# HIPS/DESI-MCMC

Hardware: AMD Instinct MI355X
Metric: source-pixel evals/sec + full-field log-lik ms, 10k sources x 5 bands x 2048^2 (higher is better)
Workload: dtype f64

## Files before the change

### desi-mcmc_amd/csrc/celeste_hip.hip

```cpp

#include <hip/hip_runtime.h>
#include <hip/hip_ext.h>

#include <cmath>
#include <cstdarg>
#include <cstddef>
#include <cstdint>
#include <cstdio>
#include <cstring>
#include <algorithm>
#include <atomic>
#include <memory>
#include <new>
#include <vector>
#include <type_traits>

#include "../../include/celeste_hip.h"
#include "host_buf.h"

static thread_local char g_err[512] = "";

static int fail(int code, const char *fmt, ...) {
    va_list ap;
    va_start(ap, fmt);
    vsnprintf(g_err, sizeof(g_err), fmt, ap);
    va_end(ap);
    return code;
}

#define HIP_TRY(expr)                                                                         \
    do {                                                                                      \
        hipError_t e_ = (expr);                                                               \
        if (e_ != hipSuccess) {                                                               \
            (void)hipDeviceSynchronize();                                                     \
            return fail(e_ == hipErrorOutOfMemory ? CEL_ERR_NOMEM : CEL_ERR_HIP, "%s: %s (%s:%d)", \
                        #expr, hipGetErrorString(e_), __FILE__, __LINE__);                    \
        }                                                                                     \
    } while (0)

#include "device_common.h"
#include "k_prep_bin.h"
#include "k_bin2.h"
#include "k_render.h"
#include "k_render_hw.h"
#include "k_render_stars.h"
#include "k_small_stars.h"
#include "k_border.h"
#include "k_render_qw.h"
#include "k_misc.h"
#include "k_patch_ll.h"
#include "k_slice_gen.h"
#include "k_estep.h"
#include "k_grad.h"
#include "k_split.h"
#include "k_slice.h"

struct Prof {
    static const int PAIRS = 1024;
    hipEvent_t *ev = nullptr;
    int kid[PAIRS];
    int head = 0, count = 0;
    double sum_ms[CEL_K_COUNT] = {0};
    int64_t n[CEL_K_COUNT] = {0};
    unsigned seen[CEL_K_COUNT] = {0};
};

enum ScratchSlot {
    SCR_PLL_BOXES,
    SCR_OFFSETS,
    SCR_VALUES,
    SCR_PATCH_DATA,
    SCR_TMP_A,
    SCR_TMP_B,
    SCR_TMP_C,
    SCR_HOST_IO,
    SCR_COUNT
};
static_assert(SCR_COUNT == 8, "eight scratch slots");

union MailShared {
    unsigned long long bin_coarse[2];
    int64_t scan_total;
    int slice_flags[12];
    struct {
        unsigned long long flags_[3];
        unsigned long long slice_bytes;
        double field_stats[2];
    } w;
};
struct Mailbox {
    double ll_band[MAX_BANDS];
    unsigned long long bin_fine[2];
    MailShared sh;
    int slice_flags1[12];
    int mass_todo;
    int unused_[3];
};
static_assert(sizeof(Mailbox) == sizeof(double) * (MAX_BANDS + 16), "the mailbox is MAX_BANDS + 16 doubles");
static_assert(offsetof(Mailbox, bin_fine) == sizeof(double) * MAX_BANDS && offsetof(Mailbox, sh) == sizeof(double) * (MAX_BANDS + 2) &&
              offsetof(MailShared, w.slice_bytes) == sizeof(int) * 6 && offsetof(MailShared, w.field_stats) == sizeof(double) * 4 &&
              offsetof(Mailbox, slice_flags1) == sizeof(double) * (MAX_BANDS + 8) && offsetof(Mailbox, mass_todo) == sizeof(double) * (MAX_BANDS + 14),
              "the mailbox members keep their offsets");
static_assert(offsetof(Mailbox, mass_todo) >= offsetof(Mailbox, slice_flags1) + sizeof(int) * 11 && sizeof(MailShared) <= sizeof(double) * 6,
              "the pending to-do count shares no word: flag slot 1 ends before it, the shared words before flag slot 1");

#ifndef SLICE_FUSE_DEFAULT
#define SLICE_FUSE_DEFAULT 0
#endif
struct cel_ctx {
    int device = 0;
    hipStream_t stream = nullptr;
    bool own_stream = false;
    int variant = 1;
    static bool env_tail_ok() { const char *e = getenv("CEL_TAIL_LOG"); return e && atof(e) >= 0.0 && atof(e) <= 300.0; }
    double tail_T = env_tail_ok() ? atof(getenv("CEL_TAIL_LOG")) : 32.0;
    double render_T = env_tail_ok() ? atof(getenv("CEL_TAIL_LOG")) : 24.0;
    int live = 0;
    int split_full = 0;
    int slice_fuse = SLICE_FUSE_DEFAULT;
    int incremental = (getenv("CEL_INCREMENTAL") && atoi(getenv("CEL_INCREMENTAL")) == 0) ? 0 : 1;
    int tile_parts = (getenv("CEL_TILE_PARTS") && (atoi(getenv("CEL_TILE_PARTS")) == 1 || atoi(getenv("CEL_TILE_PARTS")) == 2 || atoi(getenv("CEL_TILE_PARTS")) == 4))
                         ? atoi(getenv("CEL_TILE_PARTS")) : 0;
    int profile = 0;
    int star_tiles = (getenv("CEL_STAR_TILES") && atoi(getenv("CEL_STAR_TILES")) >= 0 && atoi(getenv("CEL_STAR_TILES")) <= 3)
                         ? atoi(getenv("CEL_STAR_TILES")) : 1;
    int n_cu = 256;
    int tile_order = 1;
    int tile_rows = 32;
    bool tile_timing = false;
    double nz_bias = getenv("CEL_NZ_BIAS") ? atof(getenv("CEL_NZ_BIAS")) : 4.0;
    int split_reuse = getenv("CEL_SPLIT_REUSE") ? std::min(std::max(atoi(getenv("CEL_SPLIT_REUSE")), 0), 2) : 2;
    bool mass_reuse_of() const { return split_reuse >= 2; }
    int nz_force = 0;
    int debug = 0;
    int tile_layout = 1;
    Prof prof;
    PinnedBuf<Mailbox> mail;
    hipEvent_t slice_ev[2] = {nullptr, nullptr};
    DevBuf<char> scratch[SCR_COUNT];
};

static int scratch_get(cel_ctx *c, ScratchSlot slot, size_t bytes, void **out) {
    if (bytes == 0) bytes = 8;
    HIP_TRY(c->scratch[slot].grow(bytes, bytes + bytes / 2 + 256, c->stream));
    *out = c->scratch[slot];
    return CEL_OK;
}

struct SourcesDeleter {
    void operator()(cel_sources *s) const { cel_sources_destroy(s); }
};

struct cel_images {
    cel_ctx *ctx = nullptr;
    int B = 0, H = 0, W = 0;
    int full_H = 0, win_y0 = 0;
    int noise_y0 = 0, noise_y1 = 0x7fffffff;
    int TW = 64, TH = 32, ntx = 0, nty = 0;
    cel_band hb[MAX_BANDS];
    DevBuf<BandDev> d_bands;
    DevBuf<double> d_nelec, d_lambda, d_partials, d_llband;
    bool have_nelec = false;
    DevBuf<double> d_slabs;
    DevBuf<int> d_part_cnt;
    DevBuf<SrcRec> d_recs;
    DevBuf<int4> d_boxes;
    DevBuf<int> d_kind;
    DevBuf<int> d_status;
    uint64_t recs_gen = 0, hbox_gen = 0;
    uint64_t lambda_gen = 0, lists_gen = 0;
    DevBuf<unsigned long long> d_massfx;
    uint64_t massfx_gen = 0;
    DevBuf<int> d_mass_todo;
    std::vector<int4> h_boxes;
    std::vector<int> h_status;
    DevBuf<int> d_tile_cnt, d_tile_nstar, d_tile_work, d_order;
    DevBuf<int> d_tile_cost;
    int64_t cost_S = -1;
    bool bin_two_level = false;
    int64_t mass_pending = -1;
    int64_t mass_todo_S = -1;
    uint64_t mass_gen = 0;
    const int *mass_todo_ptr = nullptr;
    double *d_mass = nullptr;
    DevBuf<long long> d_btot;
    bool nelec_u16 = false;
    bool star_one_segment = false;
    int64_t order_S = -1;
    hipEvent_t ev_step = nullptr;
    DevBuf<int64_t> d_tile_off;
    unsigned long long *d_cursor = nullptr;
    DevBuf<int> d_lists;
    int nsx = 0, nsy = 0;
    DevBuf<int> d_sup_cnt;
    DevBuf<int64_t> d_sup_off;
    DevBuf<int> d_clist;
    DevBuf<unsigned long long> d_timing;
    DevBuf<int> d_samp;
    bool ssum_valid = false;
    PinnedBuf<double> h_ssum;
    PinnedBuf<int64_t> h_soff;
    bool hsum_valid = false;
    DevBuf<NzEntry> d_nzlist;
    bool nz_valid = false;
    DevBuf<double> d_rate;
    bool rate_in_lambda = false;
    DevBuf<int4> d_sbox;
    DevBuf<int4> d_snz;
    DevBuf<int64_t> d_soff;
    DevBuf<double> d_ssum;
    DevBuf<int> d_nnz, d_nzmode;
    DevBuf<int64_t> d_nzoff;
    int64_t samp_S = 0, samp_total = 0;
    DevBuf<double> d_stats;
    DevBuf<char> d_slice;
    std::unique_ptr<cel_sources, SourcesDeleter> slice_prop;
    DevBuf<char> d_sgen;
    std::unique_ptr<cel_sources, SourcesDeleter> sgen_prop;
    int64_t last_S = 0;
    double last_entries = 0;
    bool counted = false;
    bool nelec_shared = false;
    uint64_t partials_gen = 0;
    uint64_t lambda_uid = 0;
    double lambda_T = -1.0;
    int lambda_parts = 0;
    DevBuf<int> d_dirty;
    int64_t last_dirty = -1;
    MappedBuf<double> h_small;
    double *d_small = nullptr;
    DevBuf<double> d_small_consts;
    unsigned long long small_seq = 0;
    bool llband_on_host = false;
    double h_llband[MAX_BANDS] = {0};
    bool small_off = false;
};

static std::atomic<uint64_t> g_source_gen{0};

struct cel_sources {
    cel_ctx *ctx = nullptr;
    bool counted = false;
    int64_t cap = 0, S = 0;
    int B = 0;
    uint64_t gen = 0;
    uint64_t uid = 0;
    uint64_t full_gen = 0;
    std::vector<uint64_t> row_gen;
    int64_t n_gal = -1;
    DevBuf<int> d_type;
    DevBuf<double> d_radec, d_counts, d_shape;
    std::vector<int32_t> h_type;
};

static inline int tile_parts_of(const cel_ctx *c, const cel_images *im) {
    if (im->TW != 32 || c->variant == 0) return 1;
    if (c->tile_parts) return c->tile_parts;
    const int64_t T = (int64_t)im->B * im->ntx * im->nty;
    return T <= 512 ? 4 : (T <= 3072 ? 2 : 1);
}
static inline int tile_order_of(const cel_ctx *c, const cel_images *im) {
    return ((int64_t)im->B * im->ntx * im->nty * tile_parts_of(c, im) > 2048) ? c->tile_order : 0;
}

static bool prof_alloc(Prof &p) {
    if (p.ev) return true;
    p.ev = (hipEvent_t *)calloc(2 * Prof::PAIRS, sizeof(hipEvent_t));
    if (!p.ev) return false;
    for (int i = 0; i < 2 * Prof::PAIRS; i++)
        if (hipEventCreate(&p.ev[i]) != hipSuccess) return false;
    return true;
}
static bool prof_harvest_one(Prof &p, bool wait) {
    if (p.count == 0) return false;
    const int t = (p.head - p.count + Prof::PAIRS) % Prof::PAIRS;
    if (wait) (void)hipEventSynchronize(p.ev[2 * t + 1]);
    else if (hipEventQuery(p.ev[2 * t + 1]) != hipSuccess) return false;
    float ms = 0.f;
    if (hipEventElapsedTime(&ms, p.ev[2 * t], p.ev[2 * t + 1]) == hipSuccess) {
        p.sum_ms[p.kid[t]] += ms;
        p.n[p.kid[t]] += 1;
    }
    p.count--;
    return true;
}
static int prof_slot(cel_ctx *c, int k) {
    if (!c->profile) return -1;
    if (c->profile >= 2 && (k == CEL_K_PREP || k == CEL_K_BIN || k == CEL_K_REDUCE)) return -1;
    if (c->profile == 3 && (c->prof.seen[k]++ & 3) != 0) return -1;
    Prof &p = c->prof;
    if (!prof_alloc(p)) return -1;
    if (p.count == Prof::PAIRS) prof_harvest_one(p, true);
    else if (p.count > Prof::PAIRS / 2) { if (prof_harvest_one(p, false)) prof_harvest_one(p, false); }
    const int t = p.head;
    p.head = (p.head + 1) % Prof::PAIRS;
    p.count++;
    p.kid[t] = k;
    return 2 * t;
}
static int prof_begin(cel_ctx *c, int k) {
    const int i = prof_slot(c, k);
    if (i >= 0) (void)hipEventRecord(c->prof.ev[i], c->stream);
    return i;
}
static void prof_end(cel_ctx *c, int i) {
    if (i >= 0) (void)hipEventRecord(c->prof.ev[i + 1], c->stream);
}
#define EV0(c, i) ((i) >= 0 ? (c)->prof.ev[(i)] : (hipEvent_t) nullptr)
#define EV1(c, i) ((i) >= 0 ? (c)->prof.ev[(i) + 1] : (hipEvent_t) nullptr)
template <class T> static inline T ext_arg(const T &v) { return v; }
template <class T, unsigned F> static inline T *ext_arg(const Buf<T, F> &b) { return b.get(); }
template <class K, class... A>
static inline void ext_launch(K kernel, dim3 grid, dim3 block, hipStream_t st, hipEvent_t e0, hipEvent_t e1, const A &...a) {
// ... 159 lines not shown
    case CEL_OPT_KERNEL:
        if (v != 0.0 && v != 1.0) return fail(CEL_ERR_INVALID, "CEL_OPT_KERNEL must be 0 or 1");
        c->variant = (int)v;
        return CEL_OK;
    case CEL_OPT_TAIL_LOG:
        if (v != v) { c->tail_T = 32.0; c->render_T = 24.0; return CEL_OK; }
        if (!(v >= 0.0) || v > 300.0) return fail(CEL_ERR_INVALID, "CEL_OPT_TAIL_LOG must be in [0, 300] (NaN: the defaults)");
        c->tail_T = v;
        c->render_T = v;
        return CEL_OK;
    case CEL_OPT_TAIL_LOG_SOURCE:
        if (v != v) { c->tail_T = 32.0; return CEL_OK; }
        if (!(v >= 0.0) || v > 300.0) return fail(CEL_ERR_INVALID, "CEL_OPT_TAIL_LOG_SOURCE must be in [0, 300] (NaN: the default)");
        c->tail_T = v;
        return CEL_OK;
    case CEL_OPT_INCREMENTAL:
        if (v != 0.0 && v != 1.0) return fail(CEL_ERR_INVALID, "CEL_OPT_INCREMENTAL must be 0 or 1");
        c->incremental = (int)v;
        return CEL_OK;
    case CEL_OPT_SPLIT_FULL_BOX:
        if (v != 0.0 && v != 1.0) return fail(CEL_ERR_INVALID, "CEL_OPT_SPLIT_FULL_BOX must be 0 or 1");
        c->split_full = (int)v;
        return CEL_OK;
    case CEL_OPT_SLICE_FUSE:
        if (!(v >= 0.0 && v <= 1e9) || v != floor(v)) return fail(CEL_ERR_INVALID, "CEL_OPT_SLICE_FUSE must be 0, 1 or a block count");
        c->slice_fuse = (int)v;
        return CEL_OK;
    case CEL_OPT_TILE_PARTS:
        if (v != 0.0 && v != 1.0 && v != 2.0 && v != 4.0) return fail(CEL_ERR_INVALID, "CEL_OPT_TILE_PARTS must be 0 (by the frame's size), 1, 2 or 4");
        c->tile_parts = (int)v;
        return CEL_OK;
    case CEL_OPT_PROFILE:
        if (v != 0.0 && v != 1.0 && v != 2.0 && v != 3.0) return fail(CEL_ERR_INVALID, "CEL_OPT_PROFILE must be 0, 1, 2 or 3");
        if (v != 0.0 && !prof_alloc(c->prof)) return fail(CEL_ERR_HIP, "CEL_OPT_PROFILE: cannot create the timing events");
        c->profile = (int)v;
        return CEL_OK;
    case CEL_OPT_TILE_ORDER:
        if (v != 0.0 && v != 1.0 && v != 2.0) return fail(CEL_ERR_INVALID, "CEL_OPT_TILE_ORDER must be 0, 1 or 2");
        c->tile_order = (int)v;
        return CEL_OK;
    case CEL_OPT_TILE_ROWS:
        if (v != 32.0 && v != 64.0) return fail(CEL_ERR_INVALID, "CEL_OPT_TILE_ROWS must be 32 or 64");
        c->tile_rows = (int)v;
        return CEL_OK;
    case CEL_OPT_TILE_TIMING:
        c->tile_timing = (v != 0.0);
        return CEL_OK;
    case CEL_OPT_TILE_LAYOUT:
        if (v != 0.0 && v != 1.0 && v != 2.0) return fail(CEL_ERR_INVALID, "CEL_OPT_TILE_LAYOUT must be 0, 1 or 2");
        c->tile_layout = (int)v;
        return CEL_OK;
    case CEL_OPT_PHOTON_LISTS:
        if (v != 0.0 && v != 1.0 && v != 2.0) return fail(CEL_ERR_INVALID, "CEL_OPT_PHOTON_LISTS must be 0, 1 or 2");
        c->nz_force = (int)v;
        return CEL_OK;
    case CEL_OPT_SPLIT_REUSE:
        if (v != 0.0 && v != 1.0 && v != 2.0) return fail(CEL_ERR_INVALID, "CEL_OPT_SPLIT_REUSE must be 0, 1 or 2");
        c->split_reuse = (int)v;
        return CEL_OK;
    case CEL_OPT_STAR_TILES:
        if (v != 0.0 && v != 1.0 && v != 2.0 && v != 3.0) return fail(CEL_ERR_INVALID, "CEL_OPT_STAR_TILES must be 0, 1, 2 or 3");
        c->star_tiles = (int)v;
        return CEL_OK;
    case CEL_OPT_DEBUG:
        if (!(v >= 0.0) || v > 4095.0) return fail(CEL_ERR_INVALID, "CEL_OPT_DEBUG must be in [0, 4095]");
#ifndef CEL_ABLATE
        if (((int)v) & ~(64 | 128))
            return fail(CEL_ERR_INVALID, "CEL_OPT_DEBUG: the timing-only ablation bits exist only in a -DCEL_ABLATE build "
                                         "(make -C desi-mcmc_amd/csrc ablate); this library accepts 64 and 128");
#endif
        c->debug = (int)v;
        return CEL_OK;
    }
    return fail(CEL_ERR_INVALID, "unknown option %d", key);
}

int cel_ctx_get_option(cel_ctx *c, int key, double *v) {
    if (!c || !v) return fail(CEL_ERR_INVALID, "null argument");
    switch (key) {
    case CEL_OPT_KERNEL: *v = c->variant; return CEL_OK;
    case CEL_OPT_TAIL_LOG: *v = c->render_T; return CEL_OK;
    case CEL_OPT_TAIL_LOG_SOURCE: *v = c->tail_T; return CEL_OK;
    case CEL_OPT_TILE_PARTS: *v = c->tile_parts; return CEL_OK;
    case CEL_OPT_INCREMENTAL: *v = c->incremental; return CEL_OK;
    case CEL_OPT_SPLIT_FULL_BOX: *v = c->split_full; return CEL_OK;
    case CEL_OPT_SLICE_FUSE: *v = c->slice_fuse; return CEL_OK;
    case CEL_OPT_PROFILE: *v = (double)c->profile; return CEL_OK;
    case CEL_OPT_TILE_ORDER: *v = (double)c->tile_order; return CEL_OK;
    case CEL_OPT_TILE_ROWS: *v = c->tile_rows; return CEL_OK;
    case CEL_OPT_TILE_TIMING: *v = c->tile_timing ? 1.0 : 0.0; return CEL_OK;
    case CEL_OPT_TILE_LAYOUT: *v = c->tile_layout; return CEL_OK;
    case CEL_OPT_PHOTON_LISTS: *v = c->nz_force; return CEL_OK;
    case CEL_OPT_STAR_TILES: *v = c->star_tiles; return CEL_OK;
    case CEL_OPT_SPLIT_REUSE: *v = c->split_reuse; return CEL_OK;
    case CEL_OPT_DEBUG: *v = c->debug; return CEL_OK;
    }
    return fail(CEL_ERR_INVALID, "unknown option %d", key);
}

int cel_images_destroy(cel_images *im) {
    if (!im) return CEL_OK;
    (void)hipSetDevice(im->ctx->device);
    (void)hipStreamSynchronize(im->ctx->stream);
    if (im->ev_step) (void)hipEventDestroy(im->ev_step);
    if (im->counted) im->ctx->live--;
    delete im;
    return CEL_OK;
}

int cel_images_create(cel_ctx *c, int B, int H, int W, const cel_band *bands, cel_images **out) {
    if (!c || !bands || !out) return fail(CEL_ERR_INVALID, "cel_images_create: null argument");
    if (B < 1 || B > MAX_BANDS) return fail(CEL_ERR_INVALID, "B=%d out of range [1,%d]", B, MAX_BANDS);
    if (H < 1 || W < 1 || (int64_t)H * W > (int64_t)1 << 34) return fail(CEL_ERR_INVALID, "bad image size %dx%d", H, W);
    HIP_TRY(hipSetDevice(c->device));
    std::unique_ptr<cel_images> im(new (std::nothrow) cel_images());
    if (!im) return fail(CEL_ERR_NOMEM, "out of host memory");
    im->ctx = c; im->B = B; im->H = H; im->W = W;
    im->full_H = H; im->win_y0 = 0;
    if (c->tile_layout == 1) { im->TW = HW_TW; im->TH = HW_TH; }
    else if (c->tile_layout == 2) { im->TW = QW_TW; im->TH = QW_TH; }
    else { im->TW = TILE_W; im->TH = c->tile_rows; }
    im->ntx = (W + im->TW - 1) / im->TW;
    im->nty = (H + im->TH - 1) / im->TH;
    im->nsx = (W + SUPER_W - 1) / SUPER_W;
    im->nsy = (H + SUPER_H - 1) / SUPER_H;
    BandDev hb[MAX_BANDS];
    for (int b = 0; b < B; b++) {
        im->hb[b] = bands[b];
        for (int k = 0; k < K_PSF; k++) {
            const double *cv = bands[b].cov + 4 * k;
            double det = cv[0] * cv[3] - cv[1] * cv[2];
            if (!(cv[0] > 0) || !(cv[3] > 0) || !(det > 0))
                return fail(CEL_ERR_INVALID, "band %d: PSF component %d covariance is not positive definite", b, k);
        }
        if (!(im->hb[b].R > 0.0))
            im->hb[b].R = host_bounding_radius(bands[b].mu, bands[b].cov, K_PSF, 0.001, nullptr);
        band_to_dev(im->hb[b], hb[b]);
    }
    im->star_one_segment = true;
    for (int b = 0; b < B; b++)
        for (int k = 0; k < K_PSF; k++) {
            const BandDev &d = hb[b];
            const double inv = 1.0 / (d.cxx[k] * d.cyy[k] - d.cxy[k] * d.cxy[k]);
            const double rb_ = d.R + 2.0;
            const double emax = 0.5 * quad_max_rect_hw(d.cyy[k] * inv, -d.cxy[k] * inv, d.cxx[k] * inv, -rb_ - d.mux[k], rb_ - d.mux[k],
                                                       -rb_ - d.muy[k], rb_ - d.muy[k]);
            if (!(emax <= 0.999 * STAR_EMAX)) im->star_one_segment = false;
        }
    const int64_t npix = (int64_t)B * H * W;
    const int T = B * im->ntx * im->nty, NS = B * im->nsx * im->nsy;
    hipStream_t st = c->stream;
    HIP_TRY(im->d_bands.grow(B, B, st));
    HIP_TRY(hipMemcpy(im->d_bands, hb, sizeof(BandDev) * B, hipMemcpyHostToDevice));
    HIP_TRY(im->d_nelec.grow(npix, npix, st));
    HIP_TRY(im->d_lambda.grow(npix, npix, st));
    HIP_TRY(im->d_partials.grow(T, T, st));
    HIP_TRY(im->d_llband.grow(MAX_BANDS + 4, MAX_BANDS + 4, st));
    im->d_cursor = reinterpret_cast<unsigned long long *>(im->d_llband + MAX_BANDS);
    HIP_TRY(im->d_tile_cnt.grow(T, T, st));
    HIP_TRY(im->d_tile_nstar.grow(T, T, st));
    HIP_TRY(im->d_tile_work.grow(T, T, st));
    HIP_TRY(im->d_tile_cost.grow(T, T, st));
    HIP_TRY(im->d_order.grow(T, T, st));
    HIP_TRY(im->d_tile_off.grow(T, T, st));
    HIP_TRY(im->d_sup_cnt.grow(NS, NS, st));
    HIP_TRY(im->d_sup_off.grow(NS, NS, st));
    HIP_TRY(im->d_stats.grow(2, 2, st));
    HIP_TRY(hipMemsetAsync(im->d_lambda, 0, sizeof(double) * npix, st));
    im->counted = true;
    c->live++;
    *out = im.release();
    return CEL_OK;
}

int cel_images_set_nelec(cel_images *im, const double *nelec, int mem) {
    if (!im || !nelec) return fail(CEL_ERR_INVALID, "cel_images_set_nelec: null argument");
    HIP_TRY(hipSetDevice(im->ctx->device));
    int rc = copy_in(im->d_nelec, nelec, sizeof(double) * (size_t)im->B * im->H * im->W, mem, im->ctx->stream);
    if (rc != CEL_OK) return rc;
    im->have_nelec = true;
    im->partials_gen = 0;
    im->nelec_u16 = false;
    {
        const int NB = 512;
        DevBuf<double> d_rng;
        HIP_TRY(d_rng.grow(3 * NB, 3 * NB, im->ctx->stream));
        hipLaunchKernelGGL(k_nelec_range, dim3(NB), dim3(256), 0, im->ctx->stream, (const double *)im->d_nelec,
                           (int64_t)im->B * im->H * im->W, d_rng);
        std::vector<double> h((size_t)3 * NB);
        HIP_TRY(hipMemcpyAsync(h.data(), d_rng, sizeof(double) * 3 * NB, hipMemcpyDeviceToHost, im->ctx->stream));
        HIP_TRY(hipStreamSynchronize(im->ctx->stream));
        double lo = INFINITY, hi = -INFINITY, bad = 0.0;
        for (int k = 0; k < NB; k++) { lo = fmin(lo, h[3 * k]); hi = fmax(hi, h[3 * k + 1]); bad += h[3 * k + 2]; }
        im->nelec_u16 = (bad == 0.0) && (lo >= 0.0) && (hi <= 65535.0);
    }
    return CEL_OK;
}

int cel_images_set_epsilon(cel_images *im, int band, double eps) {
    if (!im || band < 0 || band >= im->B) return fail(CEL_ERR_INVALID, "cel_images_set_epsilon: bad band");
    HIP_TRY(hipSetDevice(im->ctx->device));
    im->hb[band].eps = eps;
    im->lambda_gen = 0;
    im->partials_gen = 0;
    hipLaunchKernelGGL(k_set_eps, dim3(1), dim3(1), 0, im->ctx->stream, im->d_bands, band, eps);
    HIP_TRY(hipGetLastError());
    return CEL_OK;
}

int cel_images_set_window(cel_images *im, int y0, int full_H) {
    if (!im) return fail(CEL_ERR_INVALID, "null images");
    if (y0 < 0 || full_H < 1 || (int64_t)y0 + im->H > full_H)
        return fail(CEL_ERR_INVALID, "window rows [%d, %d) do not fit a %d-row frame", y0, y0 + im->H, full_H);
    im->win_y0 = y0;
    im->full_H = full_H;
    im->recs_gen = im->hbox_gen = 0;
    im->lambda_gen = im->lists_gen = 0;
    im->massfx_gen = 0;
    return CEL_OK;
}

int cel_images_set_noise_rows(cel_images *im, int y0, int y1) {
    if (!im) return fail(CEL_ERR_INVALID, "null images");
    if (y0 < 0 || y1 < y0) return fail(CEL_ERR_INVALID, "cel_images_set_noise_rows: rows [%d, %d)", y0, y1);
    im->noise_y0 = y0;
    im->noise_y1 = y1;
    return CEL_OK;
}

int cel_images_get_band(cel_images *im, int band, cel_band *out) {
    if (!im || !out || band < 0 || band >= im->B) return fail(CEL_ERR_INVALID, "cel_images_get_band: bad argument");
    *out = im->hb[band];
    return CEL_OK;
}

int cel_images_get_lambda(cel_images *im, double *out, int mem) {
    if (!im || !out) return fail(CEL_ERR_INVALID, "cel_images_get_lambda: null argument");
    HIP_TRY(hipSetDevice(im->ctx->device));
    return copy_out(out, im->d_lambda, sizeof(double) * (size_t)im->B * im->H * im->W, mem, im->ctx->stream);
}

int cel_images_device_ptrs(cel_images *im, void **nelec, void **lambda) {
    if (!im) return fail(CEL_ERR_INVALID, "null images");
    if (nelec) {
        *nelec = im->d_nelec; im->nelec_u16 = false; im->nelec_shared = true; im->partials_gen = 0;
    }
    if (lambda) *lambda = im->d_lambda;
    return CEL_OK;
}

int cel_images_loglik_device(cel_images *im, void **ll_band) {
    if (!im || !ll_band) return fail(CEL_ERR_INVALID, "cel_images_loglik_device: null argument");
    if (im->llband_on_host) {
        cel_ctx *c = im->ctx;
        HIP_TRY(hipSetDevice(c->device));
        HIP_TRY(hipMemcpyAsync(im->d_llband, im->h_llband, sizeof(double) * im->B, hipMemcpyHostToDevice, c->stream));
        HIP_TRY(hipStreamSynchronize(c->stream));
        im->llband_on_host = false;
    }
    *ll_band = im->d_llband;
    return CEL_OK;
}

int cel_sources_destroy(cel_sources *s) {
    if (!s) return CEL_OK;
    (void)hipSetDevice(s->ctx->device);
    (void)hipStreamSynchronize(s->ctx->stream);
    if (s->counted) s->ctx->live--;
    delete s;
    return CEL_OK;
}

int cel_sources_create(cel_ctx *c, int64_t capacity, int B, cel_sources **out) {
    if (!c || !out) return fail(CEL_ERR_INVALID, "cel_sources_create: null argument");
    if (capacity < 1 || capacity > ((int64_t)1 << 30)) return fail(CEL_ERR_INVALID, "bad capacity");
    if (B < 1 || B > MAX_BANDS) return fail(CEL_ERR_INVALID, "B=%d out of range", B);
    HIP_TRY(hipSetDevice(c->device));
    std::unique_ptr<cel_sources> s(new (std::nothrow) cel_sources());
    if (!s) return fail(CEL_ERR_NOMEM, "out of host memory");
    s->ctx = c; s->cap = capacity; s->B = B;
    s->uid = ++g_source_gen;
    HIP_TRY(s->d_type.grow(capacity, capacity, c->stream));
    HIP_TRY(s->d_radec.grow(2 * capacity, 2 * capacity, c->stream));
    HIP_TRY(s->d_counts.grow(B * capacity, B * capacity, c->stream));
    HIP_TRY(s->d_shape.grow(4 * capacity, 4 * capacity, c->stream));
    s->counted = true;
    s->ctx->live++;
    *out = s.release();
    return CEL_OK;
}

int cel_sources_set(cel_sources *s, int64_t S, const int32_t *type, const double *radec,
                    const double *counts, const double *shape, int mem) {
    if (!s || !type || !radec || !counts || !shape) return fail(CEL_ERR_INVALID, "cel_sources_set: null argument");
    if (S < 0 || S > s->cap) return fail(CEL_ERR_INVALID, "S=%lld exceeds capacity %lld", (long long)S, (long long)s->cap);
    HIP_TRY(hipSetDevice(s->ctx->device));
    hipStream_t st = s->ctx->stream;
    if (S > 0) {
        const hipMemcpyKind kind = (mem == CEL_DEVICE) ? hipMemcpyDeviceToDevice : hipMemcpyHostToDevice;
        HIP_TRY(hipMemcpyAsync(s->d_type, type, sizeof(int) * S, kind, st));
        HIP_TRY(hipMemcpyAsync(s->d_radec, radec, sizeof(double) * 2 * S, kind, st));
        HIP_TRY(hipMemcpyAsync(s->d_counts, counts, sizeof(double) * s->B * S, kind, st));
        HIP_TRY(hipMemcpyAsync(s->d_shape, shape, sizeof(double) * 4 * S, kind, st));
        if (mem != CEL_DEVICE) HIP_TRY(hipStreamSynchronize(st));
    }
    s->S = S;
    s->gen = s->full_gen = ++g_source_gen;
    s->row_gen.clear();
    s->n_gal = -1;
    s->h_type.clear();
    if (mem != CEL_DEVICE) {
        s->n_gal = 0;
        for (int64_t i = 0; i < S; i++) s->n_gal += (type[i] != 0);
        s->h_type.assign(type, type + S);
    }
    return CEL_OK;
}

int cel_sources_get(cel_sources *s, int32_t *type, double *radec, double *counts, double *shape) {
    if (!s) return fail(CEL_ERR_INVALID, "cel_sources_get: null argument");
    HIP_TRY(hipSetDevice(s->ctx->device));
    hipStream_t st = s->ctx->stream;
    const int64_t S = s->S;
    if (S > 0) {
        if (type) HIP_TRY(hipMemcpyAsync(type, s->d_type, sizeof(int) * S, hipMemcpyDeviceToHost, st));
        if (radec) HIP_TRY(hipMemcpyAsync(radec, s->d_radec, sizeof(double) * 2 * S, hipMemcpyDeviceToHost, st));
        if (counts) HIP_TRY(hipMemcpyAsync(counts, s->d_counts, sizeof(double) * s->B * S, hipMemcpyDeviceToHost, st));
        if (shape) HIP_TRY(hipMemcpyAsync(shape, s->d_shape, sizeof(double) * 4 * S, hipMemcpyDeviceToHost, st));
        HIP_TRY(hipStreamSynchronize(st));
    }
    return CEL_OK;
}

int cel_sources_set_rows(cel_sources *s, int64_t n, const int32_t *idx, const int32_t *type, const double *radec,
                         const double *counts, const double *shape) {
    if (!s || n < 0 || (n > 0 && (!idx || !type || !radec || !counts || !shape)))
        return fail(CEL_ERR_INVALID, "cel_sources_set_rows: null argument");
    for (int64_t i = 0; i < n; i++)
        if (idx[i] < 0 || idx[i] >= s->S) return fail(CEL_ERR_INVALID, "cel_sources_set_rows: row %d outside the catalogue's %lld", idx[i], (long long)s->S);
    if (n == 0) return CEL_OK;
    {
        std::vector<int32_t> seen(idx, idx + n);
        std::sort(seen.begin(), seen.end());
        for (int64_t i = 1; i < n; i++)
            if (seen[i] == seen[i - 1]) return fail(CEL_ERR_INVALID, "cel_sources_set_rows: row %d is named twice", seen[i]);
    }
    cel_ctx *c = s->ctx;
    HIP_TRY(hipSetDevice(c->device));
    hipStream_t st = c->stream;
    const int B = s->B;
    const size_t ints = ((size_t)(2 * n) * sizeof(int) + 7) & ~(size_t)7;
    const size_t bytes = ints + sizeof(double) * (size_t)n * (2 + B + 4);
    char *d = nullptr;
    int rc = scratch_get(c, SCR_HOST_IO, bytes, (void **)&d);
    if (rc) return rc;
    std::vector<char> h(bytes);
    memcpy(h.data(), idx, sizeof(int) * n);
    memcpy(h.data() + sizeof(int) * n, type, sizeof(int) * n);
    double *hd = reinterpret_cast<double *>(h.data() + ints);
    memcpy(hd, radec, sizeof(double) * 2 * n);
    memcpy(hd + 2 * n, counts, sizeof(double) * B * n);
    memcpy(hd + (2 + B) * n, shape, sizeof(double) * 4 * n);
    HIP_TRY(hipMemcpyAsync(d, h.data(), bytes, hipMemcpyHostToDevice, st));
    const double *dd = reinterpret_cast<const double *>(d + ints);
    hipLaunchKernelGGL(k_scatter_rows, dim3((unsigned)((n + 255) / 256)), dim3(256), 0, st, n, B, (const int *)d, (const int *)d + n,
                       dd, dd + 2 * n, dd + (2 + B) * n, s->d_type, s->d_radec, s->d_counts, s->d_shape);
    HIP_TRY(hipGetLastError());
    HIP_TRY(hipStreamSynchronize(st));
    if ((int64_t)s->h_type.size() == s->S) {
        for (int64_t i = 0; i < n; i++) {
            s->n_gal += (type[i] != 0) - (s->h_type[idx[i]] != 0);
            s->h_type[idx[i]] = type[i];
        }
    } else {
        s->n_gal = -1;
    }
    s->gen = ++g_source_gen;
    if ((int64_t)s->row_gen.size() != s->S) s->row_gen.assign((size_t)s->S, 0);
    for (int64_t i = 0; i < n; i++) s->row_gen[idx[i]] = s->gen;
    return CEL_OK;
}

static int ensure_recs(cel_images *im, int64_t n) {
    if (n <= im->d_recs.cap) return CEL_OK;
    im->recs_gen = im->hbox_gen = 0;
    const int64_t cap = n + n / 4 + 64;
    HIP_TRY(grow_group(im->ctx->stream, im->d_boxes, cap, im->d_kind, cap, im->d_status, cap, im->d_recs, cap));
    return CEL_OK;
}

static double rsq_galaxy() {
    double q = 1.0 - 1e-5;
    return -2.0 * log1p(-q);
}

static int run_prep(cel_images *im, cel_sources *src, const int *d_live = nullptr, int nobox = 0) {
    cel_ctx *c = im->ctx;
    int64_t n = src->S * im->B;
    int rc = ensure_recs(im, n > 0 ? n : 1);
    if (rc) return rc;
    if (n == 0) { im->recs_gen = src->gen; im->last_S = 0; return CEL_OK; }
    int pi = prof_slot(c, CEL_K_PREP);
    LAUNCH_EV(k_prep, dim3((unsigned)((n + 255) / 256)), dim3(256), c->stream, EV0(c, pi), EV1(c, pi), im->d_bands, im->B,
              im->full_H, im->W, im->win_y0, im->H, src->S, src->d_type, src->d_radec, src->d_counts, src->d_shape,
              rsq_galaxy(), im->d_recs, im->d_boxes, im->d_kind, im->d_status, im->d_cursor, d_live, nobox);
    HIP_TRY(hipGetLastError());
    im->recs_gen = (d_live || nobox) ? 0 : src->gen;
    im->last_S = src->S;
    return CEL_OK;
}

static int host_boxes(cel_images *im, cel_sources *src) {
    if (im->hbox_gen == src->gen && src->gen != 0 && im->recs_gen == src->gen) return CEL_OK;
    int rc = CEL_OK;
    if (im->recs_gen != src->gen || src->gen == 0) rc = run_prep(im, src);
    if (rc) return rc;
    const int64_t n = src->S * im->B;
    im->h_boxes.resize((size_t)n);
    im->h_status.resize((size_t)n);
    if (n) {
        hipStream_t st = im->ctx->stream;
        HIP_TRY(hipMemcpyAsync(im->h_boxes.data(), im->d_boxes, sizeof(int4) * n, hipMemcpyDeviceToHost, st));
        HIP_TRY(hipMemcpyAsync(im->h_status.data(), im->d_status, sizeof(int) * n, hipMemcpyDeviceToHost, st));
        HIP_TRY(hipStreamSynchronize(st));
    }
    im->hbox_gen = src->gen;
    return CEL_OK;
}

#define CEL_RENDER_STRICT 4
#define CEL_RENDER_KEEP_LISTS 16
static int render_impl(cel_images *im, cel_sources *src, int flags, double *ll_band, double *ll_total, double *lambda_out);

int cel_render_field(cel_images *im, cel_sources *src, int flags, double *ll_band, double *ll_total) {
    if (flags & ~(CEL_RENDER_LOGLIK | CEL_RENDER_NO_STORE)) return fail(CEL_ERR_INVALID, "cel_render_field: unknown flag bits");
    return render_impl(im, src, flags, ll_band, ll_total, nullptr);
}

static int render_small_stars(cel_images *im, cel_sources *src, int flags, bool *done) {
    cel_ctx *c = im->ctx;
    hipStream_t st = c->stream;
    const int64_t S = src->S;
    const int B = im->B;
    *done = false;
    int rc = ensure_recs(im, S * B);
    if (rc) return rc;
    const int nblk = B * im->ntx * im->nty * SMALL_NB, nblk_band = im->ntx * im->nty * SMALL_NB;
    if (!im->h_small) {
        HIP_TRY(im->h_small.grow(nblk + 1, nblk + 1, st));
        memset(im->h_small, 0, sizeof(double) * (nblk + 1));
        HIP_TRY(hipHostGetDevicePointer((void **)&im->d_small, im->h_small, 0));
        HIP_TRY(im->d_small_consts.grow(SMALL_CONSTS * B, SMALL_CONSTS * B, st));
        hipLaunchKernelGGL(k_small_consts, dim3(B), dim3(64), 0, st, (const BandDev *)im->d_bands, im->d_small_consts);
    }
    RenderArgs a;
    memset(&a, 0, sizeof(a));
    a.bands = im->d_bands; a.recs = im->d_recs; a.nelec = im->d_nelec; a.lambda = im->d_lambda; a.partials = im->d_small;
    a.S = S; a.B = B; a.H = im->H; a.W = im->W; a.ntx = im->ntx; a.nty = im->nty;
    a.flags = flags; a.variant = c->variant; a.tail_T = c->render_T;
    SmallArgs x;
    x.radec = src->d_radec; x.counts = src->d_counts;
    x.recs = im->d_recs; x.boxes = im->d_boxes; x.kind = im->d_kind; x.status = im->d_status;
    x.partials = im->d_small;
    x.flag = reinterpret_cast<unsigned long long *>(im->d_small + nblk);
    x.stamp = 0x8000000000000000ull | ++im->small_seq;
    x.full_H = im->full_H; x.win_y0 = im->win_y0;
    x.consts = im->d_small_consts;
    {
        int mul = (int)(nblk_band * 0.381966) | 1;
        auto gcd = [](int a, int b) { while (b) { int t = a % b; a = b; b = t; } return a; };
        while (mul > 1 && gcd(mul, nblk_band) != 1) mul += 2;
        if (nblk_band < 4) mul = 1;
        x.perm_mul = mul % nblk_band ? mul % nblk_band : 1;
        x.perm_add = nblk_band / 3 + 1;
    }
    x.stamps = nullptr;
    static const char *stamp_path = getenv("CEL_SMALL_STAMPS");
    DevBuf<unsigned long long> d_stamps;
    if (stamp_path) { HIP_TRY(d_stamps.grow(8 * nblk, 8 * nblk, st)); x.stamps = d_stamps; }
    int pi = prof_slot(c, CEL_K_SMALL_STARS);
    LAUNCH_EV(k_small_stars, dim3((unsigned)nblk), dim3(64 * SMALL_NWV), st, EV0(c, pi), EV1(c, pi), a, x);
    const bool ll = (flags & CEL_RENDER_LOGLIK) != 0;
    HIP_TRY(hipGetLastError());
    HIP_TRY(hipStreamSynchronize(st));
    if (d_stamps) {
        std::vector<unsigned long long> hs((size_t)8 * nblk);
        (void)hipMemcpy(hs.data(), d_stamps, sizeof(unsigned long long) * 8 * nblk, hipMemcpyDeviceToHost);
        if (FILE *fp = fopen(stamp_path, "wb")) { fwrite(hs.data(), sizeof(unsigned long long), hs.size(), fp); fclose(fp); }
    }
    unsigned long long cur0;
    memcpy(&cur0, im->h_small + nblk, sizeof(cur0));
    if (cur0 == x.stamp) { im->small_off = true; return CEL_OK; }
    if (ll) {
        for (int b = 0; b < B; b++) {
            const double *pb = im->h_small + (size_t)b * nblk_band;
            double sum[8] = {0, 0, 0, 0, 0, 0, 0, 0}, comp[8] = {0, 0, 0, 0, 0, 0, 0, 0};
            int i = 0;
            for (; i + 8 <= nblk_band; i += 8)
                for (int k = 0; k < 8; k++) {
                    const double y = pb[i + k] - comp[k];
                    const double t = sum[k] + y;
                    comp[k] = (t - sum[k]) - y;
                    sum[k] = t;
                }
            for (int k = 0; i < nblk_band; i++, k++) {
                const double y = pb[i] - comp[k];
                const double t = sum[k] + y;
                comp[k] = (t - sum[k]) - y;
                sum[k] = t;
            }
            c->mail->ll_band[b] = ((sum[0] + sum[1]) + (sum[2] + sum[3])) + ((sum[4] + sum[5]) + (sum[6] + sum[7]));
            im->h_llband[b] = c->mail->ll_band[b];
        }
        im->llband_on_host = true;
    }
    im->recs_gen = src->gen;
    im->lists_gen = 0;
    if (!(flags & CEL_RENDER_NO_STORE)) im->lambda_gen = 0;
    im->last_S = S;
    im->cost_S = -1; im->order_S = -1;
    im->last_entries = 0;
    *done = true;
    return CEL_OK;
}

struct RenderPlan {
    int flags;
    bool keep_lists, own_rows;
    int own_ty0, own_ty1;
    bool diag, stars_only;
    bool small_stars, incremental;
    int parts, parts_used;
    int tile_order;
    bool bin_direct;
};

static int plan_render(const cel_images *im, const cel_sources *src, int flags, const double *lambda_out, RenderPlan &p) {
    const cel_ctx *c = im->ctx;
    const int64_t S = src->S;
    const int T = im->B * im->ntx * im->nty;
    p.keep_lists = (flags & CEL_RENDER_KEEP_LISTS) != 0;
    p.flags = flags &= ~CEL_RENDER_KEEP_LISTS;
    p.own_rows = im->noise_y0 > 0 || im->noise_y1 < im->H;
    p.own_ty0 = 0; p.own_ty1 = im->nty;
    if (p.own_rows && (flags & CEL_RENDER_LOGLIK)) {
        if (im->noise_y0 % im->TH != 0 || (im->noise_y1 % im->TH != 0 && im->noise_y1 < im->H))
            return fail(CEL_ERR_INVALID, "the owned rows [%d, %d) must begin and end on render-tile rows (%d) for a log-likelihood",
                        im->noise_y0, im->noise_y1, im->TH);
        p.own_ty0 = im->noise_y0 / im->TH;
        p.own_ty1 = std::min(im->nty, (im->noise_y1 + im->TH - 1) / im->TH);
    }
    p.diag = c->tile_timing || (c->debug & ~64);
    const bool stars = im->TW == HW_TW && !p.diag && c->variant != 0 && src->n_gal == 0 && im->star_one_segment;
    p.stars_only = stars && c->star_tiles && (c->star_tiles == 2 || T > STAR_TILES_MIN);
    p.small_stars = stars && S > 0 && S <= SMALL_MAX_S && T <= STAR_TILES_MIN && c->star_tiles == 1 && !im->small_off && !lambda_out &&
                    !p.keep_lists && !(flags & CEL_RENDER_STRICT) && !p.own_rows;
// ... 1544 lines not shown
```

### desi-mcmc_amd/csrc/k_prep_bin.h

```cpp
#pragma once
#include "device_common.h"
__device__ inline void dev_pixel2equa(const BandDev &b, double x, double y, double cphi, double &ra,
                                      double &dec) {
    double d0 = x - b.rho[0], d1 = y - b.rho[1];
    double i0 = b.ups[0] * d0 + b.ups[1] * d1;
    double i1 = b.ups[2] * d0 + b.ups[3] * d1;
    ra = i0 / cphi + b.phi[0];
    dec = i1 + b.phi[1];
}

__device__ inline double clampd(double v, double lo, double hi) { return fmin(fmax(v, lo), hi); }

__device__ inline double comp_radius(double cxx, double cxy, double cyy, double rsq_inv, double dist) {
    double s1 = sqrt(cxx), s2 = sqrt(cyy);
    double rho = cxy / (s1 * s2);
    double A11 = s1, A21 = rho * s2, A22 = s2 * sqrt(1.0 - rho * rho);
    double An = rsq_inv * (1.0 / (A11 * A11) + (A21 * A21) / (A22 * A22));
    double Bn = rsq_inv * (-2.0 * A21 / (A11 * (A22 * A22)));
    double Cn = rsq_inv * 1.0 / (A22 * A22);
    double maj = 1.0 / sqrt(0.5 * (An + Cn - sqrt(Bn * Bn + (An - Cn) * (An - Cn))));
    return maj + dist;
}

__device__ __forceinline__ void prep_pixel(const BandDev &bd, double ra, double dec, double cphi, double &px, double &py) {
    double s0 = (ra - bd.phi[0]) * cphi, s1 = dec - bd.phi[1];
    px = (bd.ups_inv[0] * s0 + bd.ups_inv[1] * s1) + bd.rho[0];
    py = (bd.ups_inv[2] * s0 + bd.ups_inv[3] * s1) + bd.rho[1];
}

__device__ __forceinline__ void prep_star_box(const BandDev &bd, double px, double py, int H, int W, SrcRec &r) {
    const double BIG = 1073741824.0;
    bool miss = (px < -50 || px > 2.0 * H || py < -50 || px > 2.0 * W);
    if (miss || !(px == px) || !(py == py)) {
        r.type = -3;
    } else {
        double bound = bd.R;
        int lx = (int)clampd(px - bound, -BIG, BIG), hx = (int)clampd(px + bound + 1, -BIG, BIG);
        int ly = (int)clampd(py - bound, -BIG, BIG), hy = (int)clampd(py + bound + 1, -BIG, BIG);
        r.x0 = max(0, lx); r.x1 = min(hx, W);
        r.y0 = max(0, ly); r.y1 = min(hy, H);
    }
}

__device__ __forceinline__ void prep_window(SrcRec &r, double py, int win_y0, int win_h) {
    r.y0 = max(r.y0, win_y0) - win_y0;
    r.y1 = min(r.y1, win_y0 + win_h) - win_y0;
    r.py = py - (double)win_y0;
    if (r.type < 0 || r.x1 <= r.x0 || r.y1 <= r.y0) {
        r.x0 = r.x1 = r.y0 = r.y1 = 0;
        if (r.type >= 0) r.type = -1 - r.type;
    }
}

__device__ __forceinline__ void prep_store(const SrcRec &r, int64_t i, SrcRec *__restrict__ recs, int4 *__restrict__ boxes,
                                           int *__restrict__ kind, int *__restrict__ status) {
    recs[i] = r;
    boxes[i] = make_int4(r.x0, r.x1, r.y0, r.y1);
    kind[i] = r.type < 0 ? 0 : (r.type == 0 ? K_PSF : K_GAL);
    status[i] = r.type >= 0 ? 1 : (r.type == -3 ? -1 : 0);
}

struct PrepArgs {
    const BandDev *bands;
    int B, H, W, win_y0, win_h;
    int64_t S;
    const int *type;
    const double *counts, *shape;
    double rsq_gal;
    SrcRec *recs; int4 *boxes; int *kind; int *status;
    int nobox;
};
__device__ __forceinline__ void prep_one(const BandDev *__restrict__ bands, int b, int64_t s, int64_t i, int B, int H, int W, int win_y0, int win_h,
                                         const int *__restrict__ type, double ra, double dec, const double *__restrict__ counts,
                                         const double *__restrict__ shape, double rsq_gal, SrcRec *__restrict__ recs,
                                         int4 *__restrict__ boxes, int *__restrict__ kind, int *__restrict__ status, int nobox) {
    const BandDev &bd = bands[b];
    SrcRec r;
    memset(&r, 0, sizeof(r));
    int t = type[s];
    double cphi = cos(bd.phi[1] / 180.0 * PI_D);
    double px, py;
    prep_pixel(bd, ra, dec, cphi, px, py);
    r.px = px; r.py = py;
    r.scale = counts[s * B + b];
    r.type = t;
    const double BIG = 1073741824.0;
    if (t == 0) {
        prep_star_box(bd, px, py, H, W, r);
    } else if (t == 1) {
        double theta = shape[4 * s], sig = shape[4 * s + 1], phi_s = shape[4 * s + 2], rho_s = shape[4 * s + 3];
        double ra0, dec0, rax, decx, ray, decy;
        dev_pixel2equa(bd, px, py, cphi, ra0, dec0);
        dev_pixel2equa(bd, px + 10.0, py, cphi, rax, decx);
        dev_pixel2equa(bd, px, py + 10.0, cphi, ray, decy);
        double cosd = cos(dec0 * (PI_D / 180.0));
        double cd0 = (rax - ra0) / 10.0 * cosd, cd1 = (ray - ra0) / 10.0 * cosd;
        double cd2 = (decx - dec0) / 10.0, cd3 = (decy - dec0) / 10.0;
        double phi = (90.0 - phi_s) * PI_D / 180.0;
        double re_deg = fmax(1.0 / 30, sig) / 3600.0;
        double cp = cos(phi), sp = sin(phi);
        double g0 = re_deg * cp, g1 = re_deg * (sp * rho_s), g2 = re_deg * (-sp), g3 = re_deg * (cp * rho_s);
        double gd = g0 * g3 - g1 * g2;
        double gi0 = g3 / gd, gi1 = -g1 / gd, gi2 = -g2 / gd, gi3 = g0 / gd;
        double t0 = gi0 * cd0 + gi1 * cd2, t1 = gi0 * cd1 + gi1 * cd3;
        double t2 = gi2 * cd0 + gi3 * cd2, t3 = gi2 * cd1 + gi3 * cd3;
        double td = t0 * t3 - t1 * t2;
        double ti0 = t3 / td, ti1 = -t1 / td, ti2 = -t2 / td, ti3 = t0 / td;
        double w00 = ti0 * ti0 + ti1 * ti1, w01 = ti0 * ti2 + ti1 * ti3, w11 = ti2 * ti2 + ti3 * ti3;
        r.w00 = w00; r.w01 = w01; r.w11 = w11; r.theta = theta;
        double rsq_inv = 1.0 / rsq_gal;
        double bound = -INFINITY;
        if (nobox) bound = (w00 == w00 && w11 == w11) ? 4.0 * (double)(H + W) : NAN;
        for (int k = 0; k < K_PSF && !nobox; k++) {
            double mx = (px + bd.mux[k]) - px, my = (py + bd.muy[k]) - py;
            double dist = sqrt(mx * mx + my * my);
            for (int j = 0; j < K_PROF; j++) {
                double v = c_prof_var[j];
                double rr = comp_radius(v * w00 + bd.cxx[k], v * w01 + bd.cxy[k], v * w11 + bd.cyy[k],
                                        rsq_inv, dist);
                bound = fmax(bound, rr);
            }
        }
        if (!(bound == bound) || !(px == px) || !(py == py)) {
            r.type = -1;
        } else {
            r.x0 = (int)clampd(fmax(0.0, floor(px - bound)), -BIG, BIG);
            r.x1 = (int)clampd(fmin((double)W, ceil(px + bound)), -BIG, BIG);
            r.y0 = (int)clampd(fmax(0.0, floor(py - bound)), -BIG, BIG);
            r.y1 = (int)clampd(fmin((double)H, ceil(py + bound)), -BIG, BIG);
        }
    } else if (t == 2) {
        double theta = shape[4 * s], w00 = shape[4 * s + 1], w01 = shape[4 * s + 2], w11 = shape[4 * s + 3];
        r.w00 = w00; r.w01 = w01; r.w11 = w11; r.theta = theta;
        r.type = 1;
        double rsq_inv = 1.0 / rsq_gal;
        double bound = -INFINITY;
        for (int k = 0; k < K_PSF; k++) {
            double dist = sqrt(bd.mux[k] * bd.mux[k] + bd.muy[k] * bd.muy[k]);
            for (int j = 0; j < K_PROF; j++) {
                if ((j < K_EXP) ? (theta == 0.0) : (theta == 1.0)) continue;
                double v = c_prof_var[j];
                bound = fmax(bound, comp_radius(v * w00 + bd.cxx[k], v * w01 + bd.cxy[k], v * w11 + bd.cyy[k],
                                                rsq_inv, dist));
            }
        }
        if (!(bound == bound) || !(px == px) || !(py == py)) {
            r.type = -1;
        } else {
            int lx = (int)clampd(px - bound, -BIG, BIG), hx = (int)clampd(px + bound + 1, -BIG, BIG);
            int ly = (int)clampd(py - bound, -BIG, BIG), hy = (int)clampd(py + bound + 1, -BIG, BIG);
            r.x0 = max(0, lx); r.x1 = min(hx, W);
            r.y0 = max(0, ly); r.y1 = min(hy, H);
        }
    } else {
        r.type = -1;
    }
    prep_window(r, py, win_y0, win_h);
    prep_store(r, i, recs, boxes, kind, status);
}

__global__ void __launch_bounds__(256)
k_prep(const BandDev *__restrict__ bands, int B, int H, int W, int win_y0, int win_h, int64_t S,
       const int *__restrict__ type, const double *__restrict__ radec,
       const double *__restrict__ counts, const double *__restrict__ shape, double rsq_gal,
       SrcRec *__restrict__ recs, int4 *__restrict__ boxes, int *__restrict__ kind, int *__restrict__ status,
       unsigned long long *__restrict__ cursor ,
       const int *__restrict__ live ,
       int nobox = 0 ) {
    int64_t i = (int64_t)blockIdx.x * blockDim.x + threadIdx.x;
    if (i < 4 && cursor) cursor[i] = 0ull;
    if (i >= S * B) return;
    int b = (int)(i / S);
    int64_t s = i - (int64_t)b * S;
    if (live && live[s] < 0) return;
    prep_one(bands, b, s, i, B, H, W, win_y0, win_h, type, radec[2 * s], radec[2 * s + 1], counts, shape, rsq_gal, recs, boxes, kind, status, nobox);
}

__global__ void k_set_eps(BandDev *__restrict__ bands, int band, double eps) { bands[band].eps = eps; }

__global__ void __launch_bounds__(256)
k_mixture_params(int64_t N, const double *__restrict__ Wm , const double *__restrict__ v_s ,
                 const double *__restrict__ iw, const double *__restrict__ im, const double *__restrict__ ic, int Kp,
                 const double *__restrict__ amp, const double *__restrict__ sigs, int J,
                 double *__restrict__ weights, double *__restrict__ means, double *__restrict__ covars) {
    const int64_t i = (int64_t)blockIdx.x * blockDim.x + threadIdx.x;
    const int K = Kp * J;
    if (i >= N * K) return;
    const int64_t n = i / K;
    const int c = (int)(i - n * K);
    const int k = c / J, j = c - k * J;
    weights[i] = iw[k] * amp[j];
    means[2 * i + 0] = v_s[2 * n + 0] + im[2 * k + 0];
    means[2 * i + 1] = v_s[2 * n + 1] + im[2 * k + 1];
#pragma unroll
    for (int q = 0; q < 4; q++) covars[4 * i + q] = ic[4 * k + q] + sigs[j] * Wm[4 * n + q];
}

__global__ void k_stats(const SrcRec *__restrict__ recs, int64_t n, double *out) {
    int64_t i = (int64_t)blockIdx.x * blockDim.x + threadIdx.x;
    double a = 0.0, g = 0.0;
    if (i < n) {
        const SrcRec &r = recs[i];
        if (r.type >= 0) {
            a = (double)(r.x1 - r.x0) * (double)(r.y1 - r.y0);
            g = a * (r.type == 0 ? K_PSF : K_GAL);
        }
    }
    for (int o = 32; o > 0; o >>= 1) { a += __shfl_down(a, o); g += __shfl_down(g, o); }
    if ((threadIdx.x & 63) == 0 && a != 0.0) { atomicAdd(out, a); atomicAdd(out + 1, g); }
}

__global__ void __launch_bounds__(1024)
k_order(const int *__restrict__ work, int T, int *__restrict__ order) {
    __shared__ int hist[256];
    __shared__ int red[1024];
    const int tid = threadIdx.x;
    int mx = 0;
    for (int i = tid; i < T; i += 1024) mx = max(mx, work[i]);
    red[tid] = mx;
    if (tid < 256) hist[tid] = 0;
    __syncthreads();
    for (int o = 512; o > 0; o >>= 1) {
        if (tid < o) red[tid] = max(red[tid], red[tid + o]);
        __syncthreads();
    }
    const long long wmax = red[0] > 0 ? red[0] : 1;
    for (int i = tid; i < T; i += 1024) atomicAdd(&hist[255 - (int)(((long long)work[i] * 255) / wmax)], 1);
    __syncthreads();
    if (tid == 0) {
        int run = 0;
        for (int k = 0; k < 256; k++) { int c = hist[k]; hist[k] = run; run += c; }
    }
    __syncthreads();
    for (int i = tid; i < T; i += 1024) {
        int bkt = 255 - (int)(((long long)work[i] * 255) / wmax);
        order[atomicAdd(&hist[bkt], 1)] = i;
    }
}
```

Measured before the change: 354.7 billion.

## Spread galaxy bounding-radius computation across wavefront lanes in prep kernel

```diff
diff --git a/desi-mcmc_amd/csrc/celeste_hip.hip b/desi-mcmc_amd/csrc/celeste_hip.hip
--- a/desi-mcmc_amd/csrc/celeste_hip.hip
+++ b/desi-mcmc_amd/csrc/celeste_hip.hip
@@ -159,6 +159,7 @@
     int TW = 64, TH = 32, ntx = 0, nty = 0;
     cel_band hb[MAX_BANDS];
     DevBuf<BandDev> d_bands;
+    DevBuf<double> d_cphi;
     DevBuf<double> d_nelec, d_lambda, d_partials, d_llband;
     bool have_nelec = false;
     DevBuf<double> d_slabs;
@@ -624,6 +625,9 @@
     hipStream_t st = c->stream;
     HIP_TRY(im->d_bands.grow(B, B, st));
     HIP_TRY(hipMemcpy(im->d_bands, hb, sizeof(BandDev) * B, hipMemcpyHostToDevice));
+    HIP_TRY(im->d_cphi.grow(B, B, st));
+    hipLaunchKernelGGL(k_band_consts, dim3(1), dim3(MAX_BANDS), 0, st, (const BandDev *)im->d_bands, B, (double *)im->d_cphi);
+    HIP_TRY(hipGetLastError());
     HIP_TRY(im->d_nelec.grow(npix, npix, st));
     HIP_TRY(im->d_lambda.grow(npix, npix, st));
     HIP_TRY(im->d_partials.grow(T, T, st));
@@ -873,7 +877,7 @@
     if (rc) return rc;
     if (n == 0) { im->recs_gen = src->gen; im->last_S = 0; return CEL_OK; }
     int pi = prof_slot(c, CEL_K_PREP);
-    LAUNCH_EV(k_prep, dim3((unsigned)((n + 255) / 256)), dim3(256), c->stream, EV0(c, pi), EV1(c, pi), im->d_bands, im->B,
+    LAUNCH_EV(k_prep, dim3((unsigned)((n + PREP_BLOCK - 1) / PREP_BLOCK)), dim3(PREP_BLOCK), c->stream, EV0(c, pi), EV1(c, pi), im->d_bands, im->d_cphi, im->B,
               im->full_H, im->W, im->win_y0, im->H, src->S, src->d_type, src->d_radec, src->d_counts, src->d_shape,
               rsq_galaxy(), im->d_recs, im->d_boxes, im->d_kind, im->d_status, im->d_cursor, d_live, nobox);
     HIP_TRY(hipGetLastError());
diff --git a/desi-mcmc_amd/csrc/k_prep_bin.h b/desi-mcmc_amd/csrc/k_prep_bin.h
--- a/desi-mcmc_amd/csrc/k_prep_bin.h
+++ b/desi-mcmc_amd/csrc/k_prep_bin.h
@@ -49,6 +49,40 @@
     if (r.type < 0 || r.x1 <= r.x0 || r.y1 <= r.y0) {
         r.x0 = r.x1 = r.y0 = r.y1 = 0;
         if (r.type >= 0) r.type = -1 - r.type;
+    }
+}
+
+__device__ __forceinline__ void prep_gal_w(const BandDev &bd, double px, double py, double cphi, double sig, double phi_s, double rho_s,
+                                           double &w00, double &w01, double &w11) {
+    double ra0, dec0, rax, decx, ray, decy;
+    dev_pixel2equa(bd, px, py, cphi, ra0, dec0);
+    dev_pixel2equa(bd, px + 10.0, py, cphi, rax, decx);
+    dev_pixel2equa(bd, px, py + 10.0, cphi, ray, decy);
+    double cosd = cos(dec0 * (PI_D / 180.0));
+    double cd0 = (rax - ra0) / 10.0 * cosd, cd1 = (ray - ra0) / 10.0 * cosd;
+    double cd2 = (decx - dec0) / 10.0, cd3 = (decy - dec0) / 10.0;
+    double phi = (90.0 - phi_s) * PI_D / 180.0;
+    double re_deg = fmax(1.0 / 30, sig) / 3600.0;
+    double cp = cos(phi), sp = sin(phi);
+    double g0 = re_deg * cp, g1 = re_deg * (sp * rho_s), g2 = re_deg * (-sp), g3 = re_deg * (cp * rho_s);
+    double gd = g0 * g3 - g1 * g2;
+    double gi0 = g3 / gd, gi1 = -g1 / gd, gi2 = -g2 / gd, gi3 = g0 / gd;
+    double t0 = gi0 * cd0 + gi1 * cd2, t1 = gi0 * cd1 + gi1 * cd3;
+    double t2 = gi2 * cd0 + gi3 * cd2, t3 = gi2 * cd1 + gi3 * cd3;
+    double td = t0 * t3 - t1 * t2;
+    double ti0 = t3 / td, ti1 = -t1 / td, ti2 = -t2 / td, ti3 = t0 / td;
+    w00 = ti0 * ti0 + ti1 * ti1; w01 = ti0 * ti2 + ti1 * ti3; w11 = ti2 * ti2 + ti3 * ti3;
+}
+
+__device__ __forceinline__ void prep_gal_box(double px, double py, double bound, int H, int W, SrcRec &r) {
+    const double BIG = 1073741824.0;
+    if (!(bound == bound) || !(px == px) || !(py == py)) {
+        r.type = -1;
+    } else {
+        r.x0 = (int)clampd(fmax(0.0, floor(px - bound)), -BIG, BIG);
+        r.x1 = (int)clampd(fmin((double)W, ceil(px + bound)), -BIG, BIG);
+        r.y0 = (int)clampd(fmax(0.0, floor(py - bound)), -BIG, BIG);
+        r.y1 = (int)clampd(fmin((double)H, ceil(py + bound)), -BIG, BIG);
     }
 }
 
@@ -159,8 +193,57 @@
     prep_store(r, i, recs, boxes, kind, status);
 }
 
-__global__ void __launch_bounds__(256)
-k_prep(const BandDev *__restrict__ bands, int B, int H, int W, int win_y0, int win_h, int64_t S,
+#define PREP_TASK_LANES 21
+__device__ __forceinline__ double prep_wave_radii(unsigned long long m, const BandDev *__restrict__ bands, int b, double px, double py,
+                                                  double w00, double w01, double w11, double rsq_gal) {
+    const int lane = (int)(threadIdx.x & 63u);
+    const int g = lane / PREP_TASK_LANES, q = lane - g * PREP_TASK_LANES;
+    const double rsq_inv = 1.0 / rsq_gal;
+    double bound = -INFINITY;
+    while (m) {
+        const int o0 = __ffsll(m) - 1; m &= m - 1;
+        const int o1 = __ffsll(m) - 1; m &= m - 1;
+        const int o2 = __ffsll(m) - 1; m &= m - 1;
+        const int own = g == 0 ? o0 : (g == 1 ? o1 : (g == 2 ? o2 : -1));
+        const int from = own >= 0 ? own : lane;
+        const int ob = __shfl(b, from);
+        const double opx = __shfl(px, from), opy = __shfl(py, from);
+        const double o00 = __shfl(w00, from), o01 = __shfl(w01, from), o11 = __shfl(w11, from);
+        const BandDev &bd = bands[ob];
+        double v = -INFINITY;
+#pragma unroll
+        for (int h = 0; h < K_GAL / PREP_TASK_LANES; h++) {
+            const int c = q + h * PREP_TASK_LANES;
+            const int k = c / K_PROF, j = c - k * K_PROF;
+            double mx = (opx + bd.mux[k]) - opx, my = (opy + bd.muy[k]) - opy;
+            double dist = sqrt(mx * mx + my * my);
+            double pv = c_prof_var[j];
+            double rr = comp_radius(pv * o00 + bd.cxx[k], pv * o01 + bd.cxy[k], pv * o11 + bd.cyy[k], rsq_inv, dist);
+            v = fmax(v, rr);
+        }
+        for (int o = 16; o > 0; o >>= 1) {
+            double u = __shfl_down(v, o);
+            if (q + o < PREP_TASK_LANES) v = fmax(v, u);
+        }
+        const double r0 = __shfl(v, 0), r1 = __shfl(v, PREP_TASK_LANES), r2 = __shfl(v, 2 * PREP_TASK_LANES);
+        if (lane == o0) bound = r0;
+        if (lane == o1) bound = r1;
+        if (lane == o2) bound = r2;
+    }
+    return bound;
+}
+static_assert(K_GAL % PREP_TASK_LANES == 0 && 3 * PREP_TASK_LANES <= 64, "prep_wave_radii: 3 galaxies x 21 lanes x 2 components");
+
+__global__ void k_band_consts(const BandDev *__restrict__ bands, int B, double *__restrict__ cphi) {
+    int b = (int)threadIdx.x;
+    if (b < B) cphi[b] = cos(bands[b].phi[1] / 180.0 * PI_D);
+}
+
+#ifndef PREP_BLOCK
+#define PREP_BLOCK 64
+#endif
+__global__ void __launch_bounds__(PREP_BLOCK)
+k_prep(const BandDev *__restrict__ bands, const double *__restrict__ band_cphi , int B, int H, int W, int win_y0, int win_h, int64_t S,
        const int *__restrict__ type, const double *__restrict__ radec,
        const double *__restrict__ counts, const double *__restrict__ shape, double rsq_gal,
        SrcRec *__restrict__ recs, int4 *__restrict__ boxes, int *__restrict__ kind, int *__restrict__ status,
@@ -169,11 +252,39 @@
        int nobox = 0 ) {
     int64_t i = (int64_t)blockIdx.x * blockDim.x + threadIdx.x;
     if (i < 4 && cursor) cursor[i] = 0ull;
-    if (i >= S * B) return;
-    int b = (int)(i / S);
-    int64_t s = i - (int64_t)b * S;
-    if (live && live[s] < 0) return;
-    prep_one(bands, b, s, i, B, H, W, win_y0, win_h, type, radec[2 * s], radec[2 * s + 1], counts, shape, rsq_gal, recs, boxes, kind, status, nobox);
+    int b = 0;
+    int64_t s = 0;
+    bool act = i < S * B;
+    if (act) {
+        b = (int)(i / S);
+        s = i - (int64_t)b * S;
+        if (live && live[s] < 0) act = false;
+    }
+    if (nobox) {
+        if (act) prep_one(bands, b, s, i, B, H, W, win_y0, win_h, type, radec[2 * s], radec[2 * s + 1], counts, shape, rsq_gal, recs, boxes, kind, status, 1);
+        return;
+    }
+    SrcRec r;
+    memset(&r, 0, sizeof(r));
+    double px = 0.0, py = 0.0;
+    const bool gal = act && type[s] == 1;
+    if (gal) {
+        const BandDev &bd = bands[b];
+        const double cphi = band_cphi[b];
+        prep_pixel(bd, radec[2 * s], radec[2 * s + 1], cphi, px, py);
+        r.px = px; r.py = py;
+        r.scale = counts[s * B + b];
+        r.type = 1;
+        prep_gal_w(bd, px, py, cphi, shape[4 * s + 1], shape[4 * s + 2], shape[4 * s + 3], r.w00, r.w01, r.w11);
+        r.theta = shape[4 * s];
+    } else if (act) {
+        prep_one(bands, b, s, i, B, H, W, win_y0, win_h, type, radec[2 * s], radec[2 * s + 1], counts, shape, rsq_gal, recs, boxes, kind, status, 0);
+    }
+    const double bound = prep_wave_radii(__ballot(gal), bands, b, px, py, r.w00, r.w01, r.w11, rsq_gal);
+    if (!gal) return;
+    prep_gal_box(px, py, bound, H, W, r);
+    prep_window(r, py, win_y0, win_h);
+    prep_store(r, i, recs, boxes, kind, status);
 }
 
 __global__ void k_set_eps(BandDev *__restrict__ bands, int band, double eps) { bands[band].eps = eps; }
```

Result: no change. 354.4 billion (-0.1%).
